# avik-pal/LocalRegNeuralDE.jl

Hardware: NVIDIA B200
Metric: mnist_ode_train_samples_per_s (higher is better)
Workload: dtype tf32x3

## Files before the change

localregneuralde.jl_b200/csrc/lrnde_adjoint.cu:

```cuda
#include "lrnde_adjoint.h"

#include <stdio.h>
#include <stdlib.h>
#include <string.h>

#include <algorithm>

#include "lrnde_fused_dev.cuh"

enum {
  LA_ALPHA = 0,
  LA_S1 = 2,
  LA_DEL = 8,
  LA_CC = 13,
  LA_HH = 18,
  LA_EPS = 23,
  LA_DBT = 29,
  LA_HBB = 30,
  LA_HBT = 31,
  LA_NARR = 32
};

#ifdef LRNDE_UMMA_TRACE
__device__ long long g_adj_trace[1024];
#define ATRACE(row, it) do { if ((int)blockIdx.x == 1 && (it) < 16) g_adj_trace[(row) * 16 + (it)] = clock64(); } while (0)
extern "C" int lrnde_debug_trace_adj(long long* out, int n) {
  cudaMemcpyFromSymbol(out, g_adj_trace, sizeof(long long) * (size_t)n);
  return 0;
}
#else
#define ATRACE(row, it) do { } while (0)
#endif

namespace ladj {
using namespace umma;
using namespace fused;

template <int ACT>
__device__ __forceinline__ void act_pair(float x, float& h, float& s) {
  if (ACT == ACT_TANH) { h = tanhf(x); s = 1.0f - h * h; }
  else { h = lr_act(ACT, x); s = lr_dact(ACT, x); }
}

constexpr int kTapeBufs = 3;
constexpr int kTapeBufBytes = kNT * LR_ZROW * 4;
struct AChainP {
  SolveDev* S;
  int single;
  const float* Mz;
  const float* w1t;
  const float* b1;
  const float* Zx;
  const float* alpha_in;
  float* ws;
  size_t zlen;
  float* hbuf;
  uint32_t unit_bytes;
  int B, H, td, Kaug, KS, nfull, ntail, passes;
};

__device__ __forceinline__ void issue_group(uint32_t d, uint32_t a_hi, uint32_t a_lo, uint32_t b0, int nfull, int ntail,
                                            int passes, uint32_t idesc) {
  uint32_t first = 0u;
  for (int pc = 0; pc < nfull; ++pc) {
    const uint32_t bh = desc_lo(b0 + pc * 8192), bl = desc_lo(b0 + pc * 8192 + 4096);
#pragma unroll
    for (int k = 0; k < 4; ++k) {
      const uint32_t ah = a_hi + (uint32_t)((pc * 4 + k) * 8), al = a_lo + (uint32_t)((pc * 4 + k) * 8);
      if (passes == 3) {
        mma_ts(d, al, bh + 2 * k, kHi128, idesc, first);
        mma_ts(d, ah, bl + 2 * k, kHi128, idesc, 1u);
        mma_ts(d, ah, bh + 2 * k, kHi128, idesc, 1u);
      } else mma_ts(d, ah, bh + 2 * k, kHi128, idesc, first);
      first = 1u;
    }
  }
  for (int t = 0; t < ntail; ++t) {
    const uint32_t bb = b0 + nfull * 8192 + t * 2048;
    const uint32_t bh = desc_lo(bb), bl = desc_lo(bb + 1024);
    const uint32_t ah = a_hi + (uint32_t)((nfull * 4 + t) * 8), al = a_lo + (uint32_t)((nfull * 4 + t) * 8);
    if (passes == 3) {
      mma_ts(d, al, bh, kHi32, idesc, first);
      mma_ts(d, ah, bl, kHi32, idesc, 1u);
      mma_ts(d, ah, bh, kHi32, idesc, 1u);
    } else mma_ts(d, ah, bh, kHi32, idesc, first);
    first = 1u;
  }
}

template <int ACT, bool SINGLE>
__global__ void __launch_bounds__(kThreads, 1) adj_chain_kernel(AChainP p) {
  SolveDev* S = p.S;
  if (SINGLE ? S->failed : S->done) return;
  extern __shared__ uint8_t smem_raw[];
  uint8_t* smem = (uint8_t*)(((uintptr_t)smem_raw + 1023) & ~(uintptr_t)1023);
  __shared__ uint64_t a_ready, bfull[2], pdone[2], pread[2], xdone[2], out_full, tfull[kTapeBufs], tempty[kTapeBufs];
  __shared__ uint32_t tmem_slot;
  __shared__ LinComb sd[6], sy[7];
  __shared__ float s_bt[7];
  __shared__ const float* s_fh;
  __shared__ const float* s_ftape;
  __shared__ size_t s_flen, s_fzlen;
  __shared__ int s_slot, s_next;

  const int warp = __shfl_sync(0xffffffffu, (int)(threadIdx.x >> 5), 0);
  const int lane = threadIdx.x & 31;
  const int n0 = blockIdx.x * kNT;
  const int nst = SINGLE ? 1 : 6;
  const uint32_t tileB = (uint32_t)(p.nfull * 8192 + p.ntail * 2048);
  uint8_t* tC[2] = {smem, smem + tileB};
  uint8_t* tE[2] = {smem + 2 * (size_t)tileB, smem + 3 * (size_t)tileB};
  uint8_t* tbuf = smem + 4 * (size_t)tileB;

  if (threadIdx.x == 0) {
    mbar_init(&a_ready, (uint32_t)kEpiWarps);
    mbar_init(&out_full, (uint32_t)kEpiWarps);
    for (int b = 0; b < kTapeBufs; ++b) { mbar_init(&tfull[b], 1u); mbar_init(&tempty[b], (uint32_t)kEpiWarps); }
    for (int c = 0; c < 2; ++c) {
      mbar_init(&bfull[c], (uint32_t)(kEpiWarps / 2));
      mbar_init(&pdone[c], 1u);
      mbar_init(&pread[c], (uint32_t)(kEpiWarps / 2));
      mbar_init(&xdone[c], 1u);
    }
    asm volatile("fence.mbarrier_init.release.cluster;" ::: "memory");
    s_fh = S->fhtape; s_ftape = S->ftape; s_flen = S->flen; s_fzlen = S->fzlen;
    s_slot = S->slot; s_next = (S->slot + 1) % S->cap;
  }
  if (threadIdx.x >= 64 && threadIdx.x < 70) sd[threadIdx.x - 64] = S->st[threadIdx.x - 64];
  if (threadIdx.x >= 96 && threadIdx.x < 103) sy[threadIdx.x - 96] = S->yint[threadIdx.x - 96];
  if (threadIdx.x >= 128 && threadIdx.x < 135) s_bt[threadIdx.x - 128] = S->err.coef[threadIdx.x - 128];
  if (warp == 1) {
    asm volatile("tcgen05.alloc.cta_group::1.sync.aligned.shared::cta.b32 [%0], %1;" ::"r"(smem_u32(&tmem_slot)), "r"(512u)
                 : "memory");
    asm volatile("tcgen05.relinquish_alloc_permit.cta_group::1.sync.aligned;" ::: "memory");
  }
  tc_fence_before();
  __syncthreads();
  tc_fence_after();
  const uint32_t tmem_base = tmem_slot;
  const uint32_t c_acc = tmem_base + (uint32_t)(32 * p.KS);
  auto arr = [&](int idx) -> float* { return p.ws + (size_t)idx * p.zlen; };
  const bool tr = (threadIdx.x == 64) && !SINGLE;
  if (tr) ATRACE(0, 0);

  if (warp == 0) {
    {
      const int nvalid = min(kNT, p.B - n0);
      const uint32_t bytes = (uint32_t)nvalid * LR_ZROW * 4u;
      int it = 0;
      for (int jj = 0; jj < nst; ++jj) {
        const LinComb& yd = SINGLE ? sy[0] : sy[jj + 1];
        const size_t slotn = (size_t)(yd.base - s_ftape) / ((size_t)7 * s_flen);
        const float* hb = s_fh + slotn * 7 * s_fzlen;
        for (int s = 0; s < 8; ++s, ++it) {
          const int b = it % kTapeBufs;
          const float* src = (s == 7) ? hb : hb + (size_t)(s < 6 ? s + 1 : 8) * s_fzlen;
          mbar_wait(&tempty[b], (uint32_t)(((it / kTapeBufs) & 1) ^ 1));
          if (elect_one_sync()) {
            mbar_arrive_expect_tx(&tfull[b], bytes);
            bulk_g2s(tbuf + (size_t)b * kTapeBufBytes, src + (size_t)n0 * LR_ZROW, bytes, &tfull[b]);
          }
          __syncwarp();
        }
      }
    }
    if (!SINGLE) {
      mbar_wait(&out_full, 0);
      if (elect_one_sync()) {
        for (int sg = 0; sg < 4; ++sg) {
          uint8_t* g = reinterpret_cast<uint8_t*>(p.hbuf) + ((size_t)blockIdx.x * 4 + sg) * p.unit_bytes;
          const int cg = sg >> 1, half = sg & 1;
          for (int c = 0; c < p.nfull; ++c)
            for (int lo = 0; lo < 2; ++lo) {
              bulk_s2g(g + (size_t)c * 8192 + lo * 4096, tE[cg] + (size_t)c * 8192 + lo * 4096 + half * 2048, 2048);
              bulk_s2g(g + (size_t)c * 8192 + lo * 4096 + 2048, tC[cg] + (size_t)c * 8192 + lo * 4096 + half * 2048, 2048);
            }
          for (int t = 0; t < p.ntail; ++t)
            for (int lo = 0; lo < 2; ++lo) {
              const size_t o = (size_t)p.nfull * 8192 + (size_t)t * 2048 + lo * 1024;
              bulk_s2g(g + o, tE[cg] + o + half * 512, 512);
              bulk_s2g(g + o + 512, tC[cg] + o + half * 512, 512);
            }
        }
        bulk_commit();
        bulk_wait0();
      }
      __syncwarp();
    }
  } else if (warp == 1) {
    constexpr uint32_t idesc = make_idesc(128, kNT / 2);
    mbar_wait(&a_ready, 0);
    tc_fence_after();
    const uint32_t mz_hi = tmem_base, mz_lo = tmem_base + (uint32_t)(8 * p.KS);
    const uint32_t mt_hi = tmem_base + (uint32_t)(16 * p.KS), mt_lo = tmem_base + (uint32_t)(24 * p.KS);
    for (int st = 0; st < nst; ++st) {
      const uint32_t ph = (uint32_t)(st & 1);
      for (int cg = 0; cg < 2; ++cg) {
        mbar_wait(&bfull[cg], ph);
        tc_fence_after();
        if (elect_one_sync()) {
          if (cg == 0 && !SINGLE) ATRACE(7, st);
          issue_group(c_acc + (uint32_t)(cg * 32), mz_hi, mz_lo, smem_u32(tC[cg]), p.nfull, p.ntail, p.passes, idesc);
          mma_commit(&pdone[cg]);
          if (cg == 0 && !SINGLE) ATRACE(8, st);
        }
        __syncwarp();
      }
      if (!SINGLE) {
        for (int cg = 0; cg < 2; ++cg) {
          mbar_wait(&pread[cg], ph);
          tc_fence_after();
          if (elect_one_sync()) {
            issue_group(c_acc + (uint32_t)(cg * 32), mt_hi, mt_lo, smem_u32(tE[cg]), p.nfull, p.ntail, p.passes, idesc);
            mma_commit(&xdone[cg]);
          }
          __syncwarp();
        }
      }
    }
  } else {
    const int q = warp & 3, sub = (warp - 2) >> 2;
    const int cg = sub >> 1;
    const int hrow = q * 32 + lane;
    const uint32_t tlane = tmem_base + ((uint32_t)(q * 32) << 16);
    const int rbase = (sub & 1) * 16;
    const int nb = n0 + cg * 32 + rbase;
    const bool rowv = hrow < p.H;
    const bool rowc = hrow < p.Kaug;
    {
#pragma unroll
      for (int j = 0; j < 4; ++j) {
        const int ks = sub + 4 * j;
        if (ks < p.KS) {
          float a1[8], a2[8], hi[8], lo[8];
#pragma unroll
          for (int e = 0; e < 8; ++e) {
            const int k = ks * 8 + e;
            a1[e] = __ldg(p.Mz + hrow * 128 + k);
            a2[e] = (rowv && k < p.H) ? __ldg(p.Mz + k * 128 + hrow) : 0.0f;
          }
#pragma unroll
          for (int e = 0; e < 8; ++e) {
            if (p.passes == 3) { hi[e] = tf32_rna(a1[e]); lo[e] = tf32_rna(a1[e] - hi[e]); }
            else { hi[e] = a1[e]; lo[e] = 0.0f; }
          }
          tmem_st8(tlane + (uint32_t)(ks * 8), hi);
          tmem_st8(tlane + (uint32_t)(8 * p.KS + ks * 8), lo);
#pragma unroll
          for (int e = 0; e < 8; ++e) {
            if (p.passes == 3) { hi[e] = tf32_rna(a2[e]); lo[e] = tf32_rna(a2[e] - hi[e]); }
            else { hi[e] = a2[e]; lo[e] = 0.0f; }
          }
          tmem_st8(tlane + (uint32_t)(16 * p.KS + ks * 8), hi);
          tmem_st8(tlane + (uint32_t)(24 * p.KS + ks * 8), lo);
        }
      }
    }
    tmem_st_wait();
    tc_fence_before();
    __syncwarp();
    if (lane == 0) mbar_arrive(&a_ready);
    if (tr) ATRACE(0, 1);

    const bool in_full = hrow < p.nfull * 32;
    const bool in_img = hrow < p.KS * 8;
    uint32_t oA, oS, oLo, osw;
    if (in_full) {
      oS = 128u; oLo = 4096u; osw = (uint32_t)(lane >> 2);
      oA = (uint32_t)(q * 8192 + (lane & 3) * 4) + (uint32_t)rbase * oS;
    } else {
      const int kt = hrow - p.nfull * 32, t = kt >> 3, kk = kt & 7;
      oS = 32u; oLo = 1024u; osw = (uint32_t)((kk >> 2) & 1);
      oA = (uint32_t)(p.nfull * 8192 + t * 2048 + (kk & 3) * 4) + (uint32_t)rbase * oS;
    }
    const uint32_t rnd = (p.passes == 3) ? 0x1000u : 0u, msk = (p.passes == 3) ? 0xFFFFE000u : 0xFFFFFFFFu;
    auto tile_put16 = [&](uint8_t* tile, const float (&val)[16]) {
      if (!in_img) return;
#pragma unroll
      for (int i = 0; i < 16; ++i) {
        const uint32_t m = in_full ? (uint32_t)(i & 7) : (uint32_t)((i >> 2) & 1);
        const uint32_t o = oA + (uint32_t)i * oS + ((osw ^ m) << 4);
        const float hi = __uint_as_float((__float_as_uint(val[i]) + rnd) & msk);
        const float lo = __uint_as_float((__float_as_uint(val[i] - hi) + rnd) & msk);
        *reinterpret_cast<float*>(tile + o) = hi;
        *reinterpret_cast<float*>(tile + o + oLo) = lo;
      }
    };
    const float w1t = (p.td && rowv && p.w1t) ? p.w1t[hrow] : 0.0f;
    const float b1 = rowv ? p.b1[hrow] : 0.0f;
    const int slot = s_slot, next = s_next;
    const float dt = sd[0].scale;
    const float* alpha_n = SINGLE ? p.alpha_in : arr(LA_ALPHA + slot);
    const size_t e0 = (size_t)nb * LR_ZROW + hrow;
    uint8_t* const tCc = tC[cg];
    uint8_t* const tEc = tE[cg];
    const float* tape_row = reinterpret_cast<const float*>(tbuf) + (cg * 32 + rbase) * LR_ZROW + hrow;

    float c[16], ep[16], dprev[16];
#pragma unroll
    for (int i = 0; i < 16; ++i) { c[i] = 0.0f; ep[i] = 0.0f; dprev[i] = 0.0f; }
    if (!SINGLE && rowv) {
      const float* d1 = arr(LA_S1 + 3 * slot + 0) + e0;
#pragma unroll
      for (int i = 0; i < 16; ++i) dprev[i] = __ldcg(d1 + (size_t)i * LR_ZROW);
    }
    float v[16], ss[16];
    for (int jj = -1; jj < nst; ++jj) {
      const LinComb& yd = SINGLE ? sy[0] : sy[jj < 0 ? 1 : jj + 1];
      const float tau = yd.t;
      const bool last = (!SINGLE && jj == 5);
      float* dst_del = SINGLE ? arr(LA_S1 + 3 * slot + 0) : (last ? arr(LA_S1 + 3 * next + 0) : arr(LA_DEL + max(jj, 0)));
      float* dst_hh = SINGLE ? arr(LA_S1 + 3 * slot + 1) : (last ? arr(LA_S1 + 3 * next + 1) : arr(LA_HH + max(jj, 0)));
      float* dst_cc = SINGLE ? arr(LA_S1 + 3 * slot + 2) : (last ? arr(LA_S1 + 3 * next + 2) : arr(LA_CC + max(jj, 0)));
      if (jj >= 0) {
        if (tr) ATRACE(1, jj);
        const float cextra = (hrow == p.Kaug) ? tau : ((hrow == p.Kaug + 1) ? 1.0f : 0.0f);
#pragma unroll
        for (int i = 0; i < 16; ++i) dst_cc[e0 + (size_t)i * LR_ZROW] = rowc ? c[i] : cextra;
        tile_put16(tCc, c);
        if (!SINGLE) {
          const float cl = sd[jj].coef[jj];
          float* dst_eps = arr(LA_EPS + jj) + e0;
#pragma unroll
          for (int i = 0; i < 16; ++i) { v[i] = fmaf(cl, dprev[i], ep[i]); dst_eps[(size_t)i * LR_ZROW] = v[i]; }
          tile_put16(tEc, v);
        }
        tc_fence_before();
        fence_proxy_async();
        __syncwarp();
        if (lane == 0) mbar_arrive(&bfull[cg]);
        if (tr) ATRACE(2, jj);
      }
      if (jj + 1 < nst) {
        const LinComb& yn = SINGLE ? sy[0] : sy[jj + 2];
#pragma unroll
        for (int i = 0; i < 16; ++i) c[i] = 0.0f;
        for (int s = 0; s < 8; ++s) {
          const int it = (jj + 1) * 8 + s;
          const int b = it % kTapeBufs;
          mbar_wait(&tfull[b], (uint32_t)((it / kTapeBufs) & 1));
          if (rowc) {
            const float* tb = tape_row + (size_t)b * (kTapeBufBytes / 4);
            const float cf = (s < 7) ? yn.coef[s] : 1.0f, sc = (s < 7) ? 1.0f : yn.scale;
#pragma unroll
            for (int i = 0; i < 16; ++i) c[i] = fmaf(cf, tb[i * LR_ZROW], sc * c[i]);
          }
          __syncwarp();
          if (lane == 0) mbar_arrive(&tempty[b]);
        }
        if (!SINGLE && jj >= 0) {
#pragma unroll
          for (int i = 0; i < 16; ++i) ep[i] = sd[jj + 1].coef[jj] * dprev[i];
          if (rowv) {
            for (int s = 0; s < jj; ++s) {
              const float* src = ((s == 0) ? arr(LA_S1 + 3 * slot + 0) : arr(LA_DEL + s - 1)) + e0;
              const float cf = sd[jj + 1].coef[s];
#pragma unroll
              for (int i = 0; i < 16; ++i) ep[i] = fmaf(cf, __ldcg(src + (size_t)i * LR_ZROW), ep[i]);
            }
          }
        }
      }
      if (jj >= 0) {
        if (tr) ATRACE(3, jj);
#pragma unroll
        for (int i = 0; i < 16; ++i) ss[i] = rowv ? __ldcg(p.Zx + e0 + (size_t)i * LR_ZROW) : 0.0f;
        mbar_wait(&pdone[cg], (uint32_t)(jj & 1));
        if (tr) ATRACE(4, jj);
        tc_fence_after();
        tmem_ld16(c_acc + ((uint32_t)(q * 32) << 16) + (uint32_t)(cg * 32 + rbase), v);
        tc_fence_before();
        __syncwarp();
        if (!SINGLE && lane == 0) mbar_arrive(&pread[cg]);
        const float hconst = (p.td && hrow == p.H) ? tau : ((hrow == p.H + p.td) ? 1.0f : 0.0f);
        const float pb = p.td ? fmaf(w1t, tau, b1) : b1;
#pragma unroll
        for (int i = 0; i < 16; ++i) {
          float h, sg;
          act_pair<ACT>(v[i] + ss[i] + pb, h, sg);
          ss[i] = rowv ? sg : 0.0f;
          dst_hh[e0 + (size_t)i * LR_ZROW] = rowv ? h : hconst;
        }
        float an[16];
#pragma unroll
        for (int i = 0; i < 16; ++i) an[i] = rowv ? __ldcg(alpha_n + e0 + (size_t)i * LR_ZROW) : 0.0f;
        if (tr) ATRACE(5, jj);
        if (!SINGLE) {
          mbar_wait(&xdone[cg], (uint32_t)(jj & 1));
          if (tr) ATRACE(6, jj);
          tc_fence_after();
          tmem_ld16(c_acc + ((uint32_t)(q * 32) << 16) + (uint32_t)(cg * 32 + rbase), v);
          tc_fence_before();
        }
        float* dst_alpha = (SINGLE ? arr(LA_ALPHA + slot) : arr(LA_ALPHA + next)) + e0;
#pragma unroll
        for (int i = 0; i < 16; ++i) {
          const float aj = SINGLE ? an[i] : fmaf(-dt, v[i], an[i]);
          dprev[i] = ss[i] * aj;
          dst_del[e0 + (size_t)i * LR_ZROW] = dprev[i];
          if (SINGLE || last) dst_alpha[(size_t)i * LR_ZROW] = rowv ? aj : 0.0f;
        }
      }
    }
    if (tr) ATRACE(0, 3);
    if (!SINGLE) {
      const LinComb& d7 = sd[5];
      auto gather3 = [&](int s0, int ns, int which, float (&t)[3][16]) {
#pragma unroll
        for (int k = 0; k < 3; ++k) {
          const int s = min(s0 + k, 6);
          const float* src = ((s == 0) ? arr(LA_S1 + 3 * slot + which)
                                       : (s == 6 ? arr(LA_S1 + 3 * next + which) : arr((which ? LA_HH : LA_DEL) + s - 1))) + e0;
#pragma unroll
          for (int i = 0; i < 16; ++i) t[k][i] = (k < ns) ? __ldcg(src + (size_t)i * LR_ZROW) : 0.0f;
        }
      };
      float t[3][16];
#pragma unroll
      for (int i = 0; i < 16; ++i) { v[i] = s_bt[6] * dprev[i]; ss[i] = 0.0f; c[i] = 0.0f; }
      for (int round = 0; round < 5; ++round) {
        const int which = round < 2 ? 0 : 1;
        const int s0 = which ? (round - 2) * 3 : round * 3;
        const int ns = which ? min(3, 7 - s0) : 3;
        if (which ? rowc : rowv) {
          gather3(s0, ns, which, t);
#pragma unroll
          for (int k = 0; k < 3; ++k) {
            const int s = min(s0 + k, 6);
            const float ct = (k < ns) ? s_bt[s] : 0.0f;
            const float cb = (k < ns && s < 6) ? d7.coef[s] : 0.0f;
#pragma unroll
            for (int i = 0; i < 16; ++i) {
              if (which) { c[i] = fmaf(cb, t[k][i], c[i]); ss[i] = fmaf(ct, t[k][i], ss[i]); }
              else v[i] = fmaf(ct, t[k][i], v[i]);
            }
          }
        }
        if (round == 1) {
          float* dbt = arr(LA_DBT) + e0;
#pragma unroll
          for (int i = 0; i < 16; ++i) dbt[(size_t)i * LR_ZROW] = v[i];
          tile_put16(tCc, v);
          fence_proxy_async();
          __syncwarp();
          if (lane == 0) mbar_arrive(&out_full);
        }
      }
      if (tr) ATRACE(0, 4);
      float* hbb = arr(LA_HBB) + e0;
      float* hbt = arr(LA_HBT) + e0;
#pragma unroll
      for (int i = 0; i < 16; ++i) {
        hbb[(size_t)i * LR_ZROW] = rowc ? c[i] : 0.0f;
        hbt[(size_t)i * LR_ZROW] = rowc ? ss[i] : 0.0f;
      }
    }
    tc_fence_before();
  }
  __syncthreads();
  if (threadIdx.x == 0 && !SINGLE) ATRACE(0, 5);
  if (warp == 1) {
    tc_fence_after();
    asm volatile("tcgen05.dealloc.cta_group::1.sync.aligned.b32 %0, %1;" ::"r"(tmem_base), "r"(512u) : "memory");
  }
}

struct PaTerm { int p_arr, q_arr; float s0, s1; int acc; };
struct PairAccP {
  SolveDev* S;
  const float* ws;
  size_t zlen;
  const float* x;
  int D, B;
  int nP, chunkP, nD, chunkD, ntile;
  float* partP; float* partX; float* partL;
  int nterm, passes;
  PaTerm term[13];
};
constexpr int kPaStageBytes = 6 * 16384;
constexpr int kPaStages = 2;
constexpr int pairacc_smem() { return kPaStages * kPaStageBytes + 1024; }

__global__ void __launch_bounds__(kThreads, 1) pairacc_kernel(PairAccP q) {
  SolveDev* S = q.S;
  if (S->done) return;
  constexpr int NS = kPaStages;
  constexpr int PT = kEpiWarps * 32;
  extern __shared__ uint8_t smem_raw[];
  uint8_t* smem = (uint8_t*)(((uintptr_t)smem_raw + 1023) & ~(uintptr_t)1023);
  __shared__ uint64_t full_bar[NS], empty_bar[NS], done_bar;
  __shared__ uint32_t tmem_slot;

  const int warp = __shfl_sync(0xffffffffu, (int)(threadIdx.x >> 5), 0);
  const int lane = threadIdx.x & 31;
  int job, tile = 0, split, b_begin, b_end, nterm;
  if ((int)blockIdx.x < q.nP) {
    job = 0; split = blockIdx.x; nterm = q.nterm;
    b_begin = split * q.chunkP; b_end = min(q.B, b_begin + q.chunkP);
  } else {
    const int b2 = (int)blockIdx.x - q.nP;
    job = 1 + b2 / (q.ntile * q.nD);
    const int rem = b2 % (q.ntile * q.nD);
    tile = rem / q.nD; split = rem % q.nD; nterm = 1;
    b_begin = split * q.chunkD; b_end = min(q.B, b_begin + q.chunkD);
  }
  const int nchunks = (b_end > b_begin) ? (b_end - b_begin + 31) / 32 : 0;
  const int niter = nterm * nchunks;
  const int slot = S->slot, next = (S->slot + 1) % S->cap;
  auto arr = [&](int code) -> const float* {
    if (code >= 0) return q.ws + (size_t)code * q.zlen;
    if (code > -10) return q.ws + (size_t)(LA_S1 + 3 * slot + (-1 - code)) * q.zlen;
    return q.ws + (size_t)(LA_S1 + 3 * next + (-10 - code)) * q.zlen;
  };

  if (threadIdx.x == 0) {
    for (int s = 0; s < NS; ++s) {
      mbar_init(&full_bar[s], (uint32_t)kEpiWarps);
      mbar_init(&empty_bar[s], 1u);
    }
    mbar_init(&done_bar, 1u);
    asm volatile("fence.mbarrier_init.release.cluster;" ::: "memory");
  }
  if (warp == 1) {
    asm volatile("tcgen05.alloc.cta_group::1.sync.aligned.shared::cta.b32 [%0], %1;" ::"r"(smem_u32(&tmem_slot)), "r"(512u)
                 : "memory");
    asm volatile("tcgen05.relinquish_alloc_permit.cta_group::1.sync.aligned;" ::: "memory");
  }
  tc_fence_before();
  __syncthreads();
  tc_fence_after();
  const uint32_t tmem_base = tmem_slot;

  if (warp == 1) {
    constexpr uint32_t idesc = make_idesc_mn(128, 128);
    uint32_t touched = 0u;
    for (int it = 0; it < niter; ++it) {
      const int s = it % NS, ph = (it / NS) & 1;
      const int ap = (job == 0) ? q.term[it / nchunks].acc : 0;
      mbar_wait(&full_bar[s], (uint32_t)ph);
      tc_fence_after();
      const uint32_t base = smem_u32(smem + (size_t)s * kPaStageBytes);
      const uint32_t p_hi = desc_lo_mn(base), p_lo = desc_lo_mn(base + 16384);
      const uint32_t q0_hi = desc_lo_mn(base + 32768), q0_lo = desc_lo_mn(base + 49152);
      const uint32_t q1_hi = desc_lo_mn(base + 65536), q1_lo = desc_lo_mn(base + 81920);
      const uint32_t d0 = tmem_base + (uint32_t)(ap * 256), d1 = d0 + 128u;
      if (elect_one_sync()) {
#pragma unroll
        for (int kg = 0; kg < 4; ++kg) {
          const uint32_t ko = (uint32_t)kg * (4096u >> 4);
          const uint32_t first = (((touched >> ap) & 1u) == 0u && kg == 0) ? 0u : 1u;
          if (q.passes == 3) {
            mma_tf32_mn<0>(d0, p_lo + ko, q0_hi + ko, idesc, first);
            mma_tf32_mn<1>(d0, p_hi + ko, q0_lo + ko, idesc, 1u);
            mma_tf32_mn<2>(d0, p_hi + ko, q0_hi + ko, idesc, 1u);
            mma_tf32_mn<0>(d1, p_lo + ko, q1_hi + ko, idesc, first);
            mma_tf32_mn<1>(d1, p_hi + ko, q1_lo + ko, idesc, 1u);
            mma_tf32_mn<2>(d1, p_hi + ko, q1_hi + ko, idesc, 1u);
          } else {
            mma_tf32_mn(d0, p_hi + ko, q0_hi + ko, idesc, first);
            mma_tf32_mn(d1, p_hi + ko, q1_hi + ko, idesc, first);
          }
        }
        mma_commit(&empty_bar[s]);
        if (it == niter - 1) mma_commit(&done_bar);
      }
      __syncwarp();
      touched |= (1u << ap);
    }
    if (niter == 0 && elect_one_sync()) mbar_arrive(&done_bar);
    __syncwarp();
  } else if (warp >= 2) {
    const int tid = threadIdx.x - 64;
    struct Ops { const float* P; long pld; int prows; const float* Q0; const float* Q1; float s0, s1; };
    auto ops_of = [&](int it) -> Ops {
      Ops o;
      if (job == 0) {
        const PaTerm& t = q.term[it / nchunks];
        o.P = arr(t.p_arr); o.pld = LR_ZROW; o.prows = LR_ZROW;
        o.Q0 = arr(t.q_arr); o.Q1 = nullptr; o.s0 = t.s0; o.s1 = t.s1;
      } else if (job == 1) {
        o.P = q.x + (size_t)tile * 128; o.pld = q.D; o.prows = q.D - tile * 128;
        o.Q0 = arr(LA_EPS + 5); o.Q1 = arr(LA_DBT); o.s0 = 1.0f; o.s1 = 1.0f;
      } else {
        o.P = lr_slot_u(S, slot) + (size_t)tile * 128; o.pld = q.D; o.prows = q.D - tile * 128;
        o.Q0 = arr(LA_HBB); o.Q1 = arr(LA_HBT); o.s0 = 1.0f; o.s1 = 1.0f;
      }
      return o;
    };
    const bool pvec = (job == 0) || ((q.D % 4 == 0) && ((((uintptr_t)q.x) & 15) == 0) &&
                                     ((((uintptr_t)lr_slot_u(S, slot)) & 15) == 0));
    float4 v[2][6];
    auto load_iter = [&](int it, float4 (&dst)[6]) {
      const Ops o = ops_of(it);
      const int ch = it % nchunks;
#pragma unroll
      for (int g = 0; g < 6; ++g) {
        const int li = tid + (g & 1) * PT;
        const int bl = li >> 5, c4 = li & 31;
        const int b = b_begin + ch * 32 + bl;
        float4 r = make_float4(0.f, 0.f, 0.f, 0.f);
        if (b < b_end) {
          if (g < 2) {
            const int row = c4 * 4;
            const float* pp = o.P + (size_t)b * o.pld + row;
            if (pvec && row + 3 < o.prows) r = __ldcg(reinterpret_cast<const float4*>(pp));
            else {
              if (row + 0 < o.prows) r.x = __ldcg(pp + 0);
              if (row + 1 < o.prows) r.y = __ldcg(pp + 1);
              if (row + 2 < o.prows) r.z = __ldcg(pp + 2);
              if (row + 3 < o.prows) r.w = __ldcg(pp + 3);
            }
          } else if (g < 4) {
            r = __ldcg(reinterpret_cast<const float4*>(o.Q0 + (size_t)b * LR_ZROW + c4 * 4));
          } else if (o.Q1) {
            r = __ldcg(reinterpret_cast<const float4*>(o.Q1 + (size_t)b * LR_ZROW + c4 * 4));
          }
        }
        dst[g] = r;
      }
    };
    if (niter > 0) load_iter(0, v[0]);
    if (niter > 1) load_iter(1, v[1]);
    for (int it0 = 0; it0 < niter; it0 += 2) {
#pragma unroll
      for (int dd = 0; dd < 2; ++dd) {
        const int it = it0 + dd;
        if (it < niter) {
          const int s = it % NS, ph = (it / NS) & 1;
          uint8_t* stage = smem + (size_t)s * kPaStageBytes;
          const Ops o = ops_of(it);
          mbar_wait(&empty_bar[s], (uint32_t)(ph ^ 1));
#pragma unroll
          for (int g = 0; g < 6; ++g) {
            const int li = tid + (g & 1) * PT;
            const int bl = li >> 5, c4 = li & 31;
            const int grp = c4 >> 3, c32 = (c4 & 7) >> 1, half = c4 & 1, k4 = bl >> 2, r = bl & 3;
            const uint32_t off = (uint32_t)((k4 * 4 + grp) * 512 + r * 128 + ((c32 ^ r) << 5) + half * 16);
            float4 xv = (g >= 4 && !o.Q1) ? v[dd][g - 2] : v[dd][g];
            const float sc = (g < 2) ? 1.0f : ((g < 4) ? o.s0 : o.s1);
            xv.x *= sc; xv.y *= sc; xv.z *= sc; xv.w *= sc;
            float4 hi, lo;
            if (q.passes == 3) {
              hi = make_float4(tf32_rna(xv.x), tf32_rna(xv.y), tf32_rna(xv.z), tf32_rna(xv.w));
              lo = make_float4(tf32_rna(xv.x - hi.x), tf32_rna(xv.y - hi.y), tf32_rna(xv.z - hi.z), tf32_rna(xv.w - hi.w));
            } else { hi = xv; lo = make_float4(0.f, 0.f, 0.f, 0.f); }
            uint8_t* img = stage + (g >> 1) * 32768;
            *reinterpret_cast<float4*>(img + off) = hi;
            *reinterpret_cast<float4*>(img + 16384 + off) = lo;
          }
          if (it + 2 < niter) load_iter(it + 2, v[dd]);
          fence_proxy_async();
          __syncwarp();
          if (lane == 0) mbar_arrive(&full_bar[s]);
        }
      }
    }
    mbar_wait(&done_bar, 0);
    tc_fence_after();
    const int quarter = (warp & 3) * 32;
    const int wgroup = (warp - 2) >> 2;
    const int mrow = quarter + lane;
    const int nacc = (job == 0) ? 4 : 2;
    float* out;
    if (job == 0) out = q.partP + (size_t)split * 4 * 16384;
    else out = (job == 1 ? q.partX : q.partL) + ((size_t)split * q.ntile + tile) * 2 * 16384;
    for (int a = 0; a < nacc; ++a) {
      for (int cb = wgroup; cb < 8; cb += kEpiWarps / 4) {
        float r[16];
        tmem_ld16(tmem_base + ((uint32_t)quarter << 16) + (uint32_t)(a * 128 + cb * 16), r);
        float4* o4 = reinterpret_cast<float4*>(out + (size_t)a * 16384 + (size_t)mrow * 128 + cb * 16);
        if (niter == 0) {
#pragma unroll
          for (int j = 0; j < 16; ++j) r[j] = 0.0f;
        }
#pragma unroll
        for (int j = 0; j < 4; ++j) o4[j] = make_float4(r[4 * j], r[4 * j + 1], r[4 * j + 2], r[4 * j + 3]);
      }
    }
    tc_fence_before();
  }
  __syncthreads();
  if (warp == 1) {
    tc_fence_after();
    asm volatile("tcgen05.dealloc.cta_group::1.sync.aligned.b32 %0, %1;" ::"r"(tmem_base), "r"(512u) : "memory");
  }
}

struct AReduceP {
  SolveDev* S;
  const float* partP; const float* partX; const float* partL;
  float* RP; float* RX; float* RL;
  int nP, nD, ntile;
};
__global__ void __launch_bounds__(256) adj_reduce_kernel(AReduceP p) {
  if (p.S->done) return;
  const size_t nP4 = 4 * 4096, nX4 = (size_t)p.ntile * 2 * 4096;
  for (size_t i = blockIdx.x * (size_t)blockDim.x + threadIdx.x; i < nP4 + 2 * nX4; i += (size_t)gridDim.x * blockDim.x) {
    float4 s = make_float4(0.f, 0.f, 0.f, 0.f);
    if (i < nP4) {
      const float4* src = reinterpret_cast<const float4*>(p.partP) + i;
#pragma unroll 8
      for (int k = 0; k < p.nP; ++k) {
        const float4 v = __ldcg(src + (size_t)k * nP4);
        s.x += v.x; s.y += v.y; s.z += v.z; s.w += v.w;
// ... 336 lines not shown
```

localregneuralde.jl_b200/csrc/lrnde_tc.cuh:

```cuda
#pragma once
#include <cuda_runtime.h>
#include <stdint.h>
#include <stdio.h>

namespace umma {

__device__ __forceinline__ uint32_t smem_u32(const void* p) {
  return (uint32_t)__cvta_generic_to_shared(p);
}
__device__ __forceinline__ void mbar_init(uint64_t* bar, uint32_t count) {
  asm volatile("mbarrier.init.shared::cta.b64 [%0], %1;" ::"r"(smem_u32(bar)), "r"(count) : "memory");
}
__device__ __forceinline__ void mbar_arrive(uint64_t* bar) {
  asm volatile("mbarrier.arrive.shared::cta.b64 _, [%0];" ::"r"(smem_u32(bar)) : "memory");
}
__device__ __forceinline__ void mbar_arrive_expect_tx(uint64_t* bar, uint32_t bytes) {
  asm volatile("mbarrier.arrive.expect_tx.shared::cta.b64 _, [%0], %1;" ::"r"(smem_u32(bar)), "r"(bytes)
               : "memory");
}
__device__ __forceinline__ void mbar_wait(uint64_t* bar, uint32_t parity) {
  uint32_t ok = 0;
  const uint32_t addr = smem_u32(bar);
#ifdef LRNDE_WATCHDOG
  const long long t0 = clock64();
#endif
  do {
    asm volatile(
        "{\n\t.reg .pred p;\n\t"
        "mbarrier.try_wait.parity.shared::cta.b64 p, [%1], %2;\n\t"
        "selp.u32 %0, 1, 0, p;\n\t}"
        : "=r"(ok)
        : "r"(addr), "r"(parity)
        : "memory");
#ifdef LRNDE_WATCHDOG
    if (!ok && clock64() - t0 > 4000000000LL) {
      printf("[lrnde watchdog] mbarrier wait timed out: block %d thread %d smem 0x%x parity %u\n", (int)blockIdx.x,
             (int)threadIdx.x, addr, parity);
      asm volatile("trap;");
    }
#endif
  } while (!ok);
}
__device__ __forceinline__ void bulk_g2s(void* smem_dst, const void* gsrc, uint32_t bytes, uint64_t* bar) {
  asm volatile("cp.async.bulk.shared::cluster.global.mbarrier::complete_tx::bytes [%0], [%1], %2, [%3];" ::"r"(
                   smem_u32(smem_dst)),
               "l"(gsrc), "r"(bytes), "r"(smem_u32(bar))
               : "memory");
}
__device__ __forceinline__ void bulk_g2s_mc(void* smem_dst, const void* gsrc, uint32_t bytes, uint64_t* bar,
                                            uint16_t mask) {
  asm volatile(
      "cp.async.bulk.shared::cluster.global.mbarrier::complete_tx::bytes.multicast::cluster [%0], [%1], %2, [%3], %4;"
      ::"r"(smem_u32(smem_dst)), "l"(gsrc), "r"(bytes), "r"(smem_u32(bar)), "h"(mask)
      : "memory");
}
__device__ __forceinline__ void cluster_sync_all() {
  asm volatile("barrier.cluster.arrive.release.aligned;\n\tbarrier.cluster.wait.acquire.aligned;" ::: "memory");
}
__device__ __forceinline__ uint32_t cluster_ctarank() {
  uint32_t r;
  asm volatile("mov.u32 %0, %%cluster_ctarank;" : "=r"(r));
  return r;
}
__device__ __forceinline__ void fence_proxy_async() { asm volatile("fence.proxy.async.shared::cta;" ::: "memory"); }
__device__ __forceinline__ void tc_fence_before() { asm volatile("tcgen05.fence::before_thread_sync;" ::: "memory"); }
__device__ __forceinline__ void tc_fence_after() { asm volatile("tcgen05.fence::after_thread_sync;" ::: "memory"); }

__device__ __forceinline__ uint64_t make_desc(uint32_t saddr) {
  uint64_t d = 0;
  d |= (uint64_t)((saddr >> 4) & 0x3FFF);
  d |= (uint64_t)1 << 16;
  d |= (uint64_t)(1024 >> 4) << 32;
  d |= (uint64_t)1 << 46;
  d |= (uint64_t)2 << 61;
  return d;
}
__host__ __device__ constexpr uint32_t make_idesc(int M, int N) {
  return (1u << 4) | (2u << 7) | (2u << 10) | ((uint32_t)(N >> 3) << 17) | ((uint32_t)(M >> 4) << 24);
}
__device__ __forceinline__ void mma_tf32(uint32_t d_tmem, uint64_t adesc, uint64_t bdesc, uint32_t idesc,
                                         uint32_t accumulate) {
  asm volatile(
      "{\n\t.reg .pred p;\n\t"
      "setp.ne.b32 p, %4, 0;\n\t"
      "tcgen05.mma.cta_group::1.kind::tf32 [%0], %1, %2, %3, p;\n\t}"
      ::"r"(d_tmem), "l"(adesc), "l"(bdesc), "r"(idesc), "r"(accumulate)
      : "memory");
}
__device__ __forceinline__ uint32_t elect_one_sync() {
  uint32_t pred = 0;
  asm volatile(
      "{\n\t.reg .b32 rx;\n\t.reg .pred px;\n\t"
      "elect.sync rx|px, %1;\n\t"
      "@px mov.s32 %0, 1;\n\t}"
      : "+r"(pred)
      : "r"(0xFFFFFFFFu));
  return pred;
}
constexpr uint32_t kDescHi = (1024u >> 4) | (1u << 14) | (2u << 29);
__device__ __forceinline__ uint32_t desc_lo(uint32_t saddr) { return ((saddr >> 4) & 0x3FFFu) | (1u << 16); }
template <int COLL = 0>
__device__ __forceinline__ void mma_tf32_lo(uint32_t d_tmem, uint32_t a_lo32, uint32_t b_lo32, uint32_t idesc,
                                            uint32_t accumulate) {
  if (COLL == 1) {
    asm volatile(
        "{\n\t.reg .pred p;\n\t.reg .b64 da, db;\n\t"
        "setp.ne.b32 p, %4, 0;\n\t"
        "mov.b64 da, {%1, %5};\n\t"
        "mov.b64 db, {%2, %5};\n\t"
        "tcgen05.mma.cta_group::1.kind::tf32.collector::a::fill [%0], da, db, %3, p;\n\t}"
        ::"r"(d_tmem), "r"(a_lo32), "r"(b_lo32), "r"(idesc), "r"(accumulate), "r"(kDescHi)
        : "memory");
  } else if (COLL == 2) {
    asm volatile(
        "{\n\t.reg .pred p;\n\t.reg .b64 da, db;\n\t"
        "setp.ne.b32 p, %4, 0;\n\t"
        "mov.b64 da, {%1, %5};\n\t"
        "mov.b64 db, {%2, %5};\n\t"
        "tcgen05.mma.cta_group::1.kind::tf32.collector::a::lastuse [%0], da, db, %3, p;\n\t}"
        ::"r"(d_tmem), "r"(a_lo32), "r"(b_lo32), "r"(idesc), "r"(accumulate), "r"(kDescHi)
        : "memory");
  } else {
    asm volatile(
        "{\n\t.reg .pred p;\n\t.reg .b64 da, db;\n\t"
        "setp.ne.b32 p, %4, 0;\n\t"
        "mov.b64 da, {%1, %5};\n\t"
        "mov.b64 db, {%2, %5};\n\t"
        "tcgen05.mma.cta_group::1.kind::tf32 [%0], da, db, %3, p;\n\t}"
        ::"r"(d_tmem), "r"(a_lo32), "r"(b_lo32), "r"(idesc), "r"(accumulate), "r"(kDescHi)
        : "memory");
  }
}
__device__ __forceinline__ void mma_commit(uint64_t* bar) {
  asm volatile("tcgen05.commit.cta_group::1.mbarrier::arrive::one.shared::cluster.b64 [%0];" ::"r"(smem_u32(bar))
               : "memory");
}
__device__ __forceinline__ void mma_commit_mc(uint64_t* bar, uint16_t mask) {
  asm volatile(
      "tcgen05.commit.cta_group::1.mbarrier::arrive::one.shared::cluster.multicast::cluster.b64 [%0], %1;"
      ::"r"(smem_u32(bar)), "h"(mask)
      : "memory");
}
__device__ __forceinline__ float tf32_rna(float x) {
  return __uint_as_float((__float_as_uint(x) + 0x1000u) & 0xFFFFE000u);
}
__host__ __device__ constexpr uint32_t make_idesc_mn(int M, int N) {
  return make_idesc(M, N) | (1u << 15) | (1u << 16);
}
constexpr uint32_t kDescHiMN = (2048u >> 4) | (1u << 14) | (1u << 29);
__device__ __forceinline__ uint32_t desc_lo_mn(uint32_t saddr) { return ((saddr >> 4) & 0x3FFFu) | ((512u >> 4) << 16); }
template <int COLL = 0>
__device__ __forceinline__ void mma_tf32_mn(uint32_t d_tmem, uint32_t a_lo32, uint32_t b_lo32, uint32_t idesc,
                                            uint32_t accumulate) {
#define LR_MMA_MN(QUAL)                                                                              \
  asm volatile(                                                                                      \
      "{\n\t.reg .pred p;\n\t.reg .b64 da, db;\n\t"                                                \
      "setp.ne.b32 p, %4, 0;\n\t"                                                                    \
      "mov.b64 da, {%1, %5};\n\t"                                                                    \
      "mov.b64 db, {%2, %5};\n\t"                                                                    \
      "tcgen05.mma.cta_group::1.kind::tf32" QUAL " [%0], da, db, %3, p;\n\t}"                         \
      ::"r"(d_tmem), "r"(a_lo32), "r"(b_lo32), "r"(idesc), "r"(accumulate), "r"(kDescHiMN)           \
      : "memory")
  if (COLL == 1) LR_MMA_MN(".collector::a::fill");
  else if (COLL == 2) LR_MMA_MN(".collector::a::lastuse");
  else LR_MMA_MN("");
#undef LR_MMA_MN
}

__device__ __forceinline__ uint32_t swz_off(int row, int c) {
  return (uint32_t)((row >> 3) * 1024 + (row & 7) * 128 + ((c ^ (row & 7)) << 4));
}

}
```

Before: 1.083 million.

## Pipeline adjoint chain MMAs, dedupe paired tape interpolation, add L2 cache hints

Splits the single per-stage barrier into separate C and E barriers and adds an xread barrier. This lets the next stage's Z-MMA be issued right after the current transpose MMA, so tensor-core work overlaps the epilogue instead of waiting for both tiles. Stages that share a tape slot are detected and interpolated in one pass, and the second result is stored and reloaded so the tape is not fetched twice. Bulk tape loads also carry L2 evict_last or evict_first hints depending on whether the slot is reused later. The trade-off is more complex barrier phase logic and extra global stores and loads for the paired coefficients.

```diff
diff --git a/localregneuralde.jl_b200/csrc/lrnde_adjoint.cu b/localregneuralde.jl_b200/csrc/lrnde_adjoint.cu
--- a/localregneuralde.jl_b200/csrc/lrnde_adjoint.cu
+++ b/localregneuralde.jl_b200/csrc/lrnde_adjoint.cu
@@ -94,7 +94,8 @@
   if (SINGLE ? S->failed : S->done) return;
   extern __shared__ uint8_t smem_raw[];
   uint8_t* smem = (uint8_t*)(((uintptr_t)smem_raw + 1023) & ~(uintptr_t)1023);
-  __shared__ uint64_t a_ready, bfull[2], pdone[2], pread[2], xdone[2], out_full, tfull[kTapeBufs], tempty[kTapeBufs];
+  __shared__ uint64_t a_ready, cfull[2], efull[2], pdone[2], pread[2], xdone[2], xread[2], out_full, tfull[kTapeBufs],
+      tempty[kTapeBufs];
   __shared__ uint32_t tmem_slot;
   __shared__ LinComb sd[6], sy[7];
   __shared__ float s_bt[7];
@@ -117,10 +118,12 @@
     mbar_init(&out_full, (uint32_t)kEpiWarps);
     for (int b = 0; b < kTapeBufs; ++b) { mbar_init(&tfull[b], 1u); mbar_init(&tempty[b], (uint32_t)kEpiWarps); }
     for (int c = 0; c < 2; ++c) {
-      mbar_init(&bfull[c], (uint32_t)(kEpiWarps / 2));
+      mbar_init(&cfull[c], (uint32_t)(kEpiWarps / 2));
+      mbar_init(&efull[c], (uint32_t)(kEpiWarps / 2));
       mbar_init(&pdone[c], 1u);
       mbar_init(&pread[c], (uint32_t)(kEpiWarps / 2));
       mbar_init(&xdone[c], 1u);
+      mbar_init(&xread[c], (uint32_t)(kEpiWarps / 2));
     }
     asm volatile("fence.mbarrier_init.release.cluster;" ::: "memory");
     s_fh = S->fhtape; s_ftape = S->ftape; s_flen = S->flen; s_fzlen = S->fzlen;
@@ -142,15 +145,25 @@
   auto arr = [&](int idx) -> float* { return p.ws + (size_t)idx * p.zlen; };
   const bool tr = (threadIdx.x == 64) && !SINGLE;
   if (tr) ATRACE(0, 0);
+  auto slot_of = [&](int k) -> size_t {
+    const LinComb& yd = SINGLE ? sy[0] : sy[k + 1];
+    return (size_t)(yd.base - s_ftape) / ((size_t)7 * s_flen);
+  };
+  uint32_t pair = 0u;
+  for (int k = 0; k + 1 < nst; ++k)
+    if (slot_of(k + 1) == slot_of(k)) { pair |= 1u << k; ++k; }
 
   if (warp == 0) {
     {
       const int nvalid = min(kNT, p.B - n0);
       const uint32_t bytes = (uint32_t)nvalid * LR_ZROW * 4u;
+      const uint64_t keep = l2_policy_evict_last(), drop = l2_policy_evict_first();
       int it = 0;
-      for (int jj = 0; jj < nst; ++jj) {
-        const LinComb& yd = SINGLE ? sy[0] : sy[jj + 1];
-        const size_t slotn = (size_t)(yd.base - s_ftape) / ((size_t)7 * s_flen);
+      for (int jj = 0; jj < nst; jj += ((pair >> jj) & 1u) ? 2 : 1) {
+        const size_t slotn = slot_of(jj);
+        bool again = false;
+        for (int j2 = jj + (((pair >> jj) & 1u) ? 2 : 1); j2 < nst; ++j2) again |= (slot_of(j2) == slotn);
+        const uint64_t pol = again ? keep : drop;
         const float* hb = s_fh + slotn * 7 * s_fzlen;
         for (int s = 0; s < 8; ++s, ++it) {
           const int b = it % kTapeBufs;
@@ -158,7 +171,7 @@
           mbar_wait(&tempty[b], (uint32_t)(((it / kTapeBufs) & 1) ^ 1));
           if (elect_one_sync()) {
             mbar_arrive_expect_tx(&tfull[b], bytes);
-            bulk_g2s(tbuf + (size_t)b * kTapeBufBytes, src + (size_t)n0 * LR_ZROW, bytes, &tfull[b]);
+            bulk_g2s_hint(tbuf + (size_t)b * kTapeBufBytes, src + (size_t)n0 * LR_ZROW, bytes, &tfull[b], pol);
           }
           __syncwarp();
         }
@@ -193,22 +206,25 @@
     tc_fence_after();
     const uint32_t mz_hi = tmem_base, mz_lo = tmem_base + (uint32_t)(8 * p.KS);
     const uint32_t mt_hi = tmem_base + (uint32_t)(16 * p.KS), mt_lo = tmem_base + (uint32_t)(24 * p.KS);
-    for (int st = 0; st < nst; ++st) {
-      const uint32_t ph = (uint32_t)(st & 1);
-      for (int cg = 0; cg < 2; ++cg) {
-        mbar_wait(&bfull[cg], ph);
-        tc_fence_after();
-        if (elect_one_sync()) {
-          if (cg == 0 && !SINGLE) ATRACE(7, st);
-          issue_group(c_acc + (uint32_t)(cg * 32), mz_hi, mz_lo, smem_u32(tC[cg]), p.nfull, p.ntail, p.passes, idesc);
-          mma_commit(&pdone[cg]);
-          if (cg == 0 && !SINGLE) ATRACE(8, st);
-        }
-        __syncwarp();
-      }
-      if (!SINGLE) {
+    auto issue_mz = [&](int st, int cg) {
+      if (st > 0) mbar_wait(&xread[cg], (uint32_t)((st - 1) & 1));
+      mbar_wait(&cfull[cg], (uint32_t)(st & 1));
+      tc_fence_after();
+      if (elect_one_sync()) {
+        if (cg == 0 && !SINGLE) ATRACE(7, st);
+        issue_group(c_acc + (uint32_t)(cg * 32), mz_hi, mz_lo, smem_u32(tC[cg]), p.nfull, p.ntail, p.passes, idesc);
+        mma_commit(&pdone[cg]);
+        if (cg == 0 && !SINGLE) ATRACE(8, st);
+      }
+      __syncwarp();
+    };
+    for (int cg = 0; cg < 2; ++cg) issue_mz(0, cg);
+    if (!SINGLE) {
+      for (int st = 0; st < nst; ++st) {
+        const uint32_t ph = (uint32_t)(st & 1);
         for (int cg = 0; cg < 2; ++cg) {
           mbar_wait(&pread[cg], ph);
+          mbar_wait(&efull[cg], ph);
           tc_fence_after();
           if (elect_one_sync()) {
             issue_group(c_acc + (uint32_t)(cg * 32), mt_hi, mt_lo, smem_u32(tE[cg]), p.nfull, p.ntail, p.passes, idesc);
@@ -216,6 +232,8 @@
           }
           __syncwarp();
         }
+        if (st + 1 < nst)
+          for (int cg = 0; cg < 2; ++cg) issue_mz(st + 1, cg);
       }
     }
   } else {
@@ -305,50 +323,110 @@
       for (int i = 0; i < 16; ++i) dprev[i] = __ldcg(d1 + (size_t)i * LR_ZROW);
     }
     float v[16], ss[16];
-    for (int jj = -1; jj < nst; ++jj) {
-      const LinComb& yd = SINGLE ? sy[0] : sy[jj < 0 ? 1 : jj + 1];
+    auto cc_of = [&](int k) -> float* {
+      return (SINGLE ? arr(LA_S1 + 3 * slot + 2) : (k == 5 ? arr(LA_S1 + 3 * next + 2) : arr(LA_CC + k))) + e0;
+    };
+    auto cextra_of = [&](int k) -> float {
+      return (hrow == p.Kaug) ? (SINGLE ? sy[0] : sy[k + 1]).t : ((hrow == p.Kaug + 1) ? 1.0f : 0.0f);
+    };
+    int tit = 0;
+    auto interp = [&](int k, bool two) {
+      const LinComb& yn = SINGLE ? sy[0] : sy[k + 1];
+      const LinComb& y2 = SINGLE ? sy[0] : sy[min(k + 2, 6)];
+      float c2[16];
+#pragma unroll
+      for (int i = 0; i < 16; ++i) { c[i] = 0.0f; c2[i] = 0.0f; }
+      for (int s = 0; s < 8; ++s, ++tit) {
+        const int b = tit % kTapeBufs;
+        mbar_wait(&tfull[b], (uint32_t)((tit / kTapeBufs) & 1));
+        if (rowc) {
+          const float* tb = tape_row + (size_t)b * (kTapeBufBytes / 4);
+          const float cf = (s < 7) ? yn.coef[s] : 1.0f, sc = (s < 7) ? 1.0f : yn.scale;
+          const float cf2 = (s < 7) ? y2.coef[s] : 1.0f, sc2 = (s < 7) ? 1.0f : y2.scale;
+#pragma unroll
+          for (int i = 0; i < 16; ++i) {
+            const float t = tb[i * LR_ZROW];
+            c[i] = fmaf(cf, t, sc * c[i]);
+            if (two) c2[i] = fmaf(cf2, t, sc2 * c2[i]);
+          }
+        }
+        __syncwarp();
+        if (lane == 0) mbar_arrive(&tempty[b]);
+      }
+      if (two) {
+        float* dst = cc_of(k + 1);
+        const float cx = cextra_of(k + 1);
+#pragma unroll
+        for (int i = 0; i < 16; ++i) dst[(size_t)i * LR_ZROW] = rowc ? c2[i] : cx;
+      }
+    };
+    auto put_c = [&](int k, bool stored) {
+      float* dst_cc = cc_of(k);
+      if (stored) {
+#pragma unroll
+        for (int i = 0; i < 16; ++i) c[i] = rowc ? __ldcg(dst_cc + (size_t)i * LR_ZROW) : 0.0f;
+      } else {
+        const float cextra = cextra_of(k);
+#pragma unroll
+        for (int i = 0; i < 16; ++i) dst_cc[(size_t)i * LR_ZROW] = rowc ? c[i] : cextra;
+      }
+      tile_put16(tCc, c);
+      fence_proxy_async();
+      __syncwarp();
+      if (lane == 0) mbar_arrive(&cfull[cg]);
+    };
+    interp(0, pair & 1u);
+    put_c(0, false);
+    if (tr) ATRACE(0, 2);
+    for (int jj = 0; jj < nst; ++jj) {
+      const LinComb& yd = SINGLE ? sy[0] : sy[jj + 1];
       const float tau = yd.t;
       const bool last = (!SINGLE && jj == 5);
-      float* dst_del = SINGLE ? arr(LA_S1 + 3 * slot + 0) : (last ? arr(LA_S1 + 3 * next + 0) : arr(LA_DEL + max(jj, 0)));
-      float* dst_hh = SINGLE ? arr(LA_S1 + 3 * slot + 1) : (last ? arr(LA_S1 + 3 * next + 1) : arr(LA_HH + max(jj, 0)));
-      float* dst_cc = SINGLE ? arr(LA_S1 + 3 * slot + 2) : (last ? arr(LA_S1 + 3 * next + 2) : arr(LA_CC + max(jj, 0)));
-      if (jj >= 0) {
-        if (tr) ATRACE(1, jj);
-        const float cextra = (hrow == p.Kaug) ? tau : ((hrow == p.Kaug + 1) ? 1.0f : 0.0f);
-#pragma unroll
-        for (int i = 0; i < 16; ++i) dst_cc[e0 + (size_t)i * LR_ZROW] = rowc ? c[i] : cextra;
-        tile_put16(tCc, c);
-        if (!SINGLE) {
-          const float cl = sd[jj].coef[jj];
-          float* dst_eps = arr(LA_EPS + jj) + e0;
-#pragma unroll
-          for (int i = 0; i < 16; ++i) { v[i] = fmaf(cl, dprev[i], ep[i]); dst_eps[(size_t)i * LR_ZROW] = v[i]; }
-          tile_put16(tEc, v);
-        }
-        tc_fence_before();
+      float* dst_del = SINGLE ? arr(LA_S1 + 3 * slot + 0) : (last ? arr(LA_S1 + 3 * next + 0) : arr(LA_DEL + jj));
+      float* dst_hh = SINGLE ? arr(LA_S1 + 3 * slot + 1) : (last ? arr(LA_S1 + 3 * next + 1) : arr(LA_HH + jj));
+      if (tr) ATRACE(1, jj);
+      if (!SINGLE) {
+        const float cl = sd[jj].coef[jj];
+        float* dst_eps = arr(LA_EPS + jj) + e0;
+#pragma unroll
+        for (int i = 0; i < 16; ++i) { v[i] = fmaf(cl, dprev[i], ep[i]); dst_eps[(size_t)i * LR_ZROW] = v[i]; }
+        tile_put16(tEc, v);
         fence_proxy_async();
         __syncwarp();
-        if (lane == 0) mbar_arrive(&bfull[cg]);
-        if (tr) ATRACE(2, jj);
-      }
+        if (lane == 0) mbar_arrive(&efull[cg]);
+      }
+      if (tr) ATRACE(2, jj);
+      float an[16];
+#pragma unroll
+      for (int i = 0; i < 16; ++i) {
+        ss[i] = rowv ? __ldcg(p.Zx + e0 + (size_t)i * LR_ZROW) : 0.0f;
+        an[i] = rowv ? __ldcg(alpha_n + e0 + (size_t)i * LR_ZROW) : 0.0f;
+      }
+      mbar_wait(&pdone[cg], (uint32_t)(jj & 1));
+      if (tr) ATRACE(4, jj);
+      tc_fence_after();
+      tmem_ld16(c_acc + ((uint32_t)(q * 32) << 16) + (uint32_t)(cg * 32 + rbase), v);
+      tc_fence_before();
+      __syncwarp();
+      if (!SINGLE && lane == 0) mbar_arrive(&pread[cg]);
+      const float hconst = (p.td && hrow == p.H) ? tau : ((hrow == p.H + p.td) ? 1.0f : 0.0f);
+      const float pb = p.td ? fmaf(w1t, tau, b1) : b1;
+#pragma unroll
+      for (int i = 0; i < 16; ++i) {
+        float h, sg;
+        act_pair<ACT>(v[i] + ss[i] + pb, h, sg);
+        ss[i] = rowv ? sg : 0.0f;
+        dst_hh[e0 + (size_t)i * LR_ZROW] = rowv ? h : hconst;
+      }
+      if (tr) ATRACE(5, jj);
       if (jj + 1 < nst) {
-        const LinComb& yn = SINGLE ? sy[0] : sy[jj + 2];
-#pragma unroll
-        for (int i = 0; i < 16; ++i) c[i] = 0.0f;
-        for (int s = 0; s < 8; ++s) {
-          const int it = (jj + 1) * 8 + s;
-          const int b = it % kTapeBufs;
-          mbar_wait(&tfull[b], (uint32_t)((it / kTapeBufs) & 1));
-          if (rowc) {
-            const float* tb = tape_row + (size_t)b * (kTapeBufBytes / 4);
-            const float cf = (s < 7) ? yn.coef[s] : 1.0f, sc = (s < 7) ? 1.0f : yn.scale;
-#pragma unroll
-            for (int i = 0; i < 16; ++i) c[i] = fmaf(cf, tb[i * LR_ZROW], sc * c[i]);
-          }
-          __syncwarp();
-          if (lane == 0) mbar_arrive(&tempty[b]);
-        }
-        if (!SINGLE && jj >= 0) {
+        if ((pair >> jj) & 1u) {
+          put_c(jj + 1, true);
+        } else {
+          interp(jj + 1, (pair >> (jj + 1)) & 1u);
+          put_c(jj + 1, false);
+        }
+        if (!SINGLE) {
 #pragma unroll
           for (int i = 0; i < 16; ++i) ep[i] = sd[jj + 1].coef[jj] * dprev[i];
           if (rowv) {
@@ -361,45 +439,23 @@
           }
         }
       }
-      if (jj >= 0) {
-        if (tr) ATRACE(3, jj);
-#pragma unroll
-        for (int i = 0; i < 16; ++i) ss[i] = rowv ? __ldcg(p.Zx + e0 + (size_t)i * LR_ZROW) : 0.0f;
-        mbar_wait(&pdone[cg], (uint32_t)(jj & 1));
-        if (tr) ATRACE(4, jj);
+      if (tr) ATRACE(3, jj);
+      if (!SINGLE) {
+        mbar_wait(&xdone[cg], (uint32_t)(jj & 1));
+        if (tr) ATRACE(6, jj);
         tc_fence_after();
         tmem_ld16(c_acc + ((uint32_t)(q * 32) << 16) + (uint32_t)(cg * 32 + rbase), v);
         tc_fence_before();
         __syncwarp();
-        if (!SINGLE && lane == 0) mbar_arrive(&pread[cg]);
-        const float hconst = (p.td && hrow == p.H) ? tau : ((hrow == p.H + p.td) ? 1.0f : 0.0f);
-        const float pb = p.td ? fmaf(w1t, tau, b1) : b1;
-#pragma unroll
-        for (int i = 0; i < 16; ++i) {
-          float h, sg;
-          act_pair<ACT>(v[i] + ss[i] + pb, h, sg);
-          ss[i] = rowv ? sg : 0.0f;
-          dst_hh[e0 + (size_t)i * LR_ZROW] = rowv ? h : hconst;
-        }
-        float an[16];
-#pragma unroll
-        for (int i = 0; i < 16; ++i) an[i] = rowv ? __ldcg(alpha_n + e0 + (size_t)i * LR_ZROW) : 0.0f;
-        if (tr) ATRACE(5, jj);
-        if (!SINGLE) {
-          mbar_wait(&xdone[cg], (uint32_t)(jj & 1));
-          if (tr) ATRACE(6, jj);
-          tc_fence_after();
-          tmem_ld16(c_acc + ((uint32_t)(q * 32) << 16) + (uint32_t)(cg * 32 + rbase), v);
-          tc_fence_before();
-        }
-        float* dst_alpha = (SINGLE ? arr(LA_ALPHA + slot) : arr(LA_ALPHA + next)) + e0;
-#pragma unroll
-        for (int i = 0; i < 16; ++i) {
-          const float aj = SINGLE ? an[i] : fmaf(-dt, v[i], an[i]);
-          dprev[i] = ss[i] * aj;
-          dst_del[e0 + (size_t)i * LR_ZROW] = dprev[i];
-          if (SINGLE || last) dst_alpha[(size_t)i * LR_ZROW] = rowv ? aj : 0.0f;
-        }
+        if (jj + 1 < nst && lane == 0) mbar_arrive(&xread[cg]);
+      }
+      float* dst_alpha = (SINGLE ? arr(LA_ALPHA + slot) : arr(LA_ALPHA + next)) + e0;
+#pragma unroll
+      for (int i = 0; i < 16; ++i) {
+        const float aj = SINGLE ? an[i] : fmaf(-dt, v[i], an[i]);
+        dprev[i] = ss[i] * aj;
+        dst_del[e0 + (size_t)i * LR_ZROW] = dprev[i];
+        if (SINGLE || last) dst_alpha[(size_t)i * LR_ZROW] = rowv ? aj : 0.0f;
       }
     }
     if (tr) ATRACE(0, 3);
diff --git a/localregneuralde.jl_b200/csrc/lrnde_tc.cuh b/localregneuralde.jl_b200/csrc/lrnde_tc.cuh
--- a/localregneuralde.jl_b200/csrc/lrnde_tc.cuh
+++ b/localregneuralde.jl_b200/csrc/lrnde_tc.cuh
@@ -46,6 +46,23 @@
                    smem_u32(smem_dst)),
                "l"(gsrc), "r"(bytes), "r"(smem_u32(bar))
                : "memory");
+}
+__device__ __forceinline__ uint64_t l2_policy_evict_last() {
+  uint64_t pol;
+  asm volatile("createpolicy.fractional.L2::evict_last.b64 %0, 1.0;" : "=l"(pol));
+  return pol;
+}
+__device__ __forceinline__ uint64_t l2_policy_evict_first() {
+  uint64_t pol;
+  asm volatile("createpolicy.fractional.L2::evict_first.b64 %0, 1.0;" : "=l"(pol));
+  return pol;
+}
+__device__ __forceinline__ void bulk_g2s_hint(void* smem_dst, const void* gsrc, uint32_t bytes, uint64_t* bar,
+                                              uint64_t policy) {
+  asm volatile(
+      "cp.async.bulk.shared::cluster.global.mbarrier::complete_tx::bytes.L2::cache_hint [%0], [%1], %2, [%3], %4;"
+      ::"r"(smem_u32(smem_dst)), "l"(gsrc), "r"(bytes), "r"(smem_u32(bar)), "l"(policy)
+      : "memory");
 }
 __device__ __forceinline__ void bulk_g2s_mc(void* smem_dst, const void* gsrc, uint32_t bytes, uint64_t* bar,
                                             uint16_t mask) {
```

New measurement: 1.110 million, median of 6. 1.02x the previous value.
